# Pearbiossom-M/FlashAttention-from-Scratch-with-Triton

Hardware: AMD Instinct MI355X
Metric: achieved TFLOPS fwd and fwd+bwd (B=4,H=32,N=4096,D=64 causal); %MFMA peak (higher is better)
Workload: dtype bf16

## Files before the change

### flashattention-from-scratch-with-triton_amd/csrc/fa_api.hip

```cpp
#include <stdint.h>
#include <stdio.h>
#include <string.h>

#include <atomic>

#include "../../include/mi355fa.h"
#include "../../include/mi355fa_local.h"
#include "../../include/mi355fa_gqa.h"
#include "../../include/mi355fa_kvcache.h"
#include "../../include/mi355fa_softcap.h"
#include "../../include/mi355fa_alibi.h"
#include "../../include/mi355fa_kvcache_fp8.h"
#include "../../include/mi355fa_sink.h"
#include "../../include/mi355fa_paged.h"
#include "../../include/mi355fa_ragged.h"
#include "fa_decode.h"
#include "fa_kernels.h"

namespace fa {
std::atomic<int> g_force_fwd{0}, g_force_dq{0}, g_force_dkv{0};
std::atomic<int> g_force_kvsplits{0};
}

namespace {

thread_local char g_err[256] = "";
void* g_dbg = nullptr;

int fail(int code, const char* fmt, const char* what) {
  snprintf(g_err, sizeof(g_err), fmt, what);
  return code;
}

int hip_fail(hipError_t e, const char* what) {
  snprintf(g_err, sizeof(g_err), "%s: %s (%d)", what, hipGetErrorString(e), (int)e);
  return (int)e;
}

bool misaligned(const void* p) { return (reinterpret_cast<uintptr_t>(p) & 15u) != 0; }

int check_scale(const char* fn, float scale) {
  uint32_t u;
  memcpy(&u, &scale, sizeof(u));
  const bool negative_or_zero = (u >> 31) != 0 || (u & 0x7fffffffu) == 0;
  const bool nan_or_inf = ((u >> 23) & 0xffu) == 0xffu;
  if (negative_or_zero || nan_or_inf) return fail(MI355FA_ERR_SHAPE, "%s: scale must be finite and > 0", fn);
  return 0;
}

int check_softcap(const char* fn, float softcap) {
  uint32_t u;
  memcpy(&u, &softcap, sizeof(u));
  const bool negative_or_zero = (u >> 31) != 0 || (u & 0x7fffffffu) == 0;
  const bool nan_or_inf = ((u >> 23) & 0xffu) == 0xffu;
  if (negative_or_zero || nan_or_inf) return fail(MI355FA_ERR_SOFTCAP, "%s: softcap must be finite and > 0", fn);
  return 0;
}

int check_common(const char* fn, int B, int H, int Sq, int Sk, int D, int dtype, bool decode = false) {
  if (B < 1 || H < 1 || Sq < 1 || Sk < 1) return fail(MI355FA_ERR_SHAPE, "%s: B, H, S_q, S_k must be >= 1", fn);
  if (D != 64 && D != 128 && !(decode && D == 256)) return fail(MI355FA_ERR_HEAD_DIM, "%s: head dim must be 64 or 128", fn);
  if (dtype != MI355FA_FP16 && dtype != MI355FA_BF16) return fail(MI355FA_ERR_DTYPE, "%s: dtype must be 0 (fp16) or 1 (bf16)", fn);
  const long long lim = (1ll << 31) - 1;
  if ((long long)Sq * D * 2 > lim || (long long)Sk * D * 2 > lim)
    return fail(MI355FA_ERR_SHAPE, "%s: one (batch, head) slice exceeds 2^31 bytes", fn);
  if ((long long)B * H * ((Sq > Sk ? Sq : Sk) + 127) / 128 > lim)
    return fail(MI355FA_ERR_SHAPE, "%s: too many tiles for one launch", fn);
  return 0;
}

int make_layout(const char* fn, const long long* st, int H, int S, int D, fa::TensorLayout* out, int out_B = 0) {
  if (!st) {
    *out = fa::contiguous_layout(H, S, D);
    return 0;
// ... 34 lines not shown
  out->seed_hi = (unsigned)(seed >> 32);
  out->offset = (unsigned)offset;
  out->rp = 256.f / (256.f - (float)thresh);
  return 0;
}

}

__global__ __launch_bounds__(256, 1) void fa_poison_kernel() {
  extern __shared__ __attribute__((aligned(16))) char poison_smem[];
  const unsigned nan2 = 0x7FC07FC0u;
  for (int i = threadIdx.x; i < 160 * 1024 / 4; i += 256) ((unsigned*)poison_smem)[i] = nan2;
#define FA_P4(n) "v_mov_b32 v" #n ", %0\n\tv_accvgpr_write_b32 a" #n ", %0\n\t"
#define FA_P16(a, b, c, d) FA_P4(a) FA_P4(b) FA_P4(c) FA_P4(d)
  asm volatile(
      FA_P16(8, 9, 10, 11) FA_P16(12, 13, 14, 15) FA_P16(16, 17, 18, 19) FA_P16(20, 21, 22, 23) FA_P16(24, 25, 26, 27) FA_P16(28, 29, 30, 31)
      FA_P16(32, 33, 34, 35) FA_P16(36, 37, 38, 39) FA_P16(40, 41, 42, 43) FA_P16(44, 45, 46, 47) FA_P16(48, 49, 50, 51) FA_P16(52, 53, 54, 55)
      FA_P16(56, 57, 58, 59) FA_P16(60, 61, 62, 63) FA_P16(64, 65, 66, 67) FA_P16(68, 69, 70, 71) FA_P16(72, 73, 74, 75) FA_P16(76, 77, 78, 79)
      FA_P16(80, 81, 82, 83) FA_P16(84, 85, 86, 87) FA_P16(88, 89, 90, 91) FA_P16(92, 93, 94, 95) FA_P16(96, 97, 98, 99) FA_P16(100, 101, 102, 103)
      FA_P16(104, 105, 106, 107) FA_P16(108, 109, 110, 111) FA_P16(112, 113, 114, 115) FA_P16(116, 117, 118, 119) FA_P16(120, 121, 122, 123)
      FA_P16(124, 125, 126, 127) FA_P16(128, 129, 130, 131) FA_P16(132, 133, 134, 135) FA_P16(136, 137, 138, 139) FA_P16(140, 141, 142, 143)
      FA_P16(144, 145, 146, 147) FA_P16(148, 149, 150, 151) FA_P16(152, 153, 154, 155) FA_P16(156, 157, 158, 159) FA_P16(160, 161, 162, 163)
      FA_P16(164, 165, 166, 167) FA_P16(168, 169, 170, 171) FA_P16(172, 173, 174, 175) FA_P16(176, 177, 178, 179) FA_P16(180, 181, 182, 183)
      FA_P16(184, 185, 186, 187) FA_P16(188, 189, 190, 191) FA_P16(192, 193, 194, 195) FA_P16(196, 197, 198, 199) FA_P16(200, 201, 202, 203)
      FA_P16(204, 205, 206, 207) FA_P16(208, 209, 210, 211) FA_P16(212, 213, 214, 215) FA_P16(216, 217, 218, 219) FA_P16(220, 221, 222, 223)
      FA_P16(224, 225, 226, 227) FA_P16(228, 229, 230, 231) FA_P16(232, 233, 234, 235) FA_P16(236, 237, 238, 239) FA_P16(240, 241, 242, 243)
      FA_P16(244, 245, 246, 247) FA_P16(248, 249, 250, 251) FA_P16(252, 253, 254, 255)
      "v_accvgpr_write_b32 a0, %0\n\tv_accvgpr_write_b32 a1, %0\n\tv_accvgpr_write_b32 a2, %0\n\tv_accvgpr_write_b32 a3, %0\n\t"
      "v_accvgpr_write_b32 a4, %0\n\tv_accvgpr_write_b32 a5, %0\n\tv_accvgpr_write_b32 a6, %0\n\tv_accvgpr_write_b32 a7, %0"
      :: "v"(nan2)
      : "memory"
#define FA_C(n) , "v" #n, "a" #n
#define FA_C8(n) FA_C(n##0) FA_C(n##1) FA_C(n##2) FA_C(n##3) FA_C(n##4) FA_C(n##5) FA_C(n##6) FA_C(n##7) FA_C(n##8) FA_C(n##9)
        , "v8", "v9", "a0", "a1", "a2", "a3", "a4", "a5", "a6", "a7", "a8", "a9"
        FA_C8(1) FA_C8(2) FA_C8(3) FA_C8(4) FA_C8(5) FA_C8(6) FA_C8(7) FA_C8(8) FA_C8(9) FA_C8(10) FA_C8(11) FA_C8(12) FA_C8(13) FA_C8(14)
        FA_C8(15) FA_C8(16) FA_C8(17) FA_C8(18) FA_C8(19) FA_C8(20) FA_C8(21) FA_C8(22) FA_C8(23) FA_C8(24)
        FA_C(250) FA_C(251) FA_C(252) FA_C(253) FA_C(254) FA_C(255));
#undef FA_C8
#undef FA_C
#undef FA_P16
#undef FA_P4
  __syncthreads();
}

extern "C" {

int fa_abi_version(void) { return MI355FA_ABI_VERSION; }

void fa_debug_force_impl(int fwd, int dq, int dkv) {
  fa::g_force_fwd.store(fwd, std::memory_order_relaxed);
  fa::g_force_dq.store(dq, std::memory_order_relaxed);
  fa::g_force_dkv.store(dkv, std::memory_order_relaxed);
}

int fa_debug_pick(int kernel, int D, int dtype, int causal, int B, int H, int S_q, int S_k) {
  if (kernel == 0) return fa::pick_fwd_impl(fa::g_force_fwd, D, dtype, B, H, S_q, S_k, causal != 0, true);
  if (kernel == 1) return fa::pick_dq_impl(fa::g_force_dq, D, dtype, B, H, S_q, S_k, causal != 0);
  return fa::pick_dkv_impl(fa::g_force_dkv, D, dtype, B, H, S_q, S_k, causal != 0);
}

int fa_debug_pick_ex(int kernel, int D, int dtype, int causal, int B, int H, int S_q, int S_k, int varlen, int contiguous,
                     int dropout) {
  (void)contiguous;
  if (kernel == 0) return fa::fwd_family(D, dtype, B, H, S_q, S_k, causal != 0, varlen != 0, dropout != 0);
  if (kernel == 1) return fa::dq_family(D, dtype, B, H, S_q, S_k, causal != 0, varlen != 0, dropout != 0);
  return fa::dkv_family(D, dtype, B, H, S_q, S_k, causal != 0, varlen != 0, dropout != 0);
}

int fa_debug_fastdiv(int n, int d) {
  const fa::FastDiv f = fa::make_fastdiv(d);
  const unsigned hi = (unsigned)(((unsigned long long)f.m * (unsigned)n) >> 32);
  return (int)((hi + (unsigned)n) >> f.l);
}

void fa_debug_set_buffer(void* p) { g_dbg = p; }

int fa_debug_poison(void* stream) {
  return (int)fa::launch_kernel<fa_poison_kernel>(2048, 256, 160 * 1024, (hipStream_t)stream);
}

void fa_debug_kvcache_splits(int n) { fa::g_force_kvsplits.store(n > 0 ? n : 0, std::memory_order_relaxed); }

const char* fa_last_error(void) { return g_err; }

int fa_supported(int D, int dtype) {
  return (D == 64 || D == 128) && (dtype == MI355FA_FP16 || dtype == MI355FA_BF16);
}

static int check_sinks(const char* fn, const float* sinks) {
  if (!sinks) return fail(MI355FA_ERR_NULL, "%s: sinks is NULL", fn);
  if (reinterpret_cast<uintptr_t>(sinks) & 3u) return fail(MI355FA_ERR_ALIGN, "%s: sinks must be 4-byte aligned", fn);
  return 0;
}

static int check_alibi(const char* fn, const float* slopes, long long stride, int B, int H) {
  if (!slopes) return fail(MI355FA_ERR_NULL, "%s: alibi_slopes is NULL", fn);
  if (reinterpret_cast<uintptr_t>(slopes) & 3u) return fail(MI355FA_ERR_ALIGN, "%s: alibi_slopes must be 4-byte aligned", fn);
  if (stride < 0 || (stride > 0 && stride < (long long)H))
    return fail(MI355FA_ERR_ALIBI, "%s: slopes_batch_stride must be 0 (shape (H,)) or >= H (shape (B, H))", fn);
  if (stride > 0 && (long long)(B > 1 ? B - 1 : 0) * stride + H > 0x7fffffffLL)
    return fail(MI355FA_ERR_ALIBI, "%s: slopes_batch_stride too large: (B - 1) * stride + H must stay below 2^31", fn);
  return 0;
}

static int make_group(const char* fn, int H, int H_kv, fa::ScoreMod* w) {
  if (H_kv < 1 || (H >= 1 && H % H_kv != 0))
// ... 796 lines not shown
```

### flashattention-from-scratch-with-triton_amd/csrc/fa_bwd_dkv_v4.hip

```cpp
#include <stdlib.h>

#include <type_traits>

#include "fa_common.h"
#include "fa_kernels.h"
#include "fa_stamps.h"

namespace fa {

struct Dkv4Cfg : Ring4Cfg<64, 128, 3> {
  static constexpr int D = 64;
  static constexpr int BK = 256, BQ = TILE_ROWS, NT = 256, NW = 4;
  static constexpr int QB = BQ / 32;
  static constexpr int ROWB = D * 2, CPR = D / 8, KS = D / 16, DB = D / 32;
  static constexpr int QBLK = 32 * ROWB;
  static constexpr int DO_BASE = NBUF * TILE_BYTES;
  static constexpr int ROWC_OFF = 2 * NBUF * TILE_BYTES;
  static constexpr int ROWC_BYTES = 2 * BQ * 4;
  static constexpr int KS_OFF = ROWC_OFF + NBUF * ROWC_BYTES;
  static constexpr int KG_BYTES = 32 * ROWB;
  static constexpr int EPI_OFF = KS_OFF + BK * ROWB;
  static constexpr int LDS_BYTES = EPI_OFF + NW * KG_BYTES;
  static constexpr int NS = 16;
  static constexpr int ACC_DV = 0, ACC_DK = 64, F_K = 16, F_V = 24, A_RC = 192;
  static constexpr int STAGE_PIECES = KG_BYTES / 1024;
  static constexpr int kStageReqs = 4 * STAGE_PIECES;
  static constexpr int kRowConstReqs = kPfLoadReqs;
  static constexpr int kPrologueReqs = 2 * kTileReqs + kRowConstReqs;
  static constexpr int kEpilogueStores = 4 * kTileRowStores<D>;
};


template <typename T, bool CAUSAL>
__global__ __launch_bounds__(256, 1) void fa_bwd_dkv4_kernel(BwdParams p) {
#ifdef FA_STAMPS
  FA_STAMPS_BEGIN(8);
  unsigned long long ntile_ = 0, npass_ = 0;
#endif
  using C = Dkv4Cfg;
  using vec8 = typename T::vec8;
  constexpr int D = C::D;
  constexpr bool FOLD = T::kFoldScale;
  extern __shared__ __attribute__((aligned(16))) char smem_raw[];
  FA_LDS char* smem = (FA_LDS char*)smem_raw;

  const int tid = threadIdx.x;
  const int wave = __builtin_amdgcn_readfirstlane(tid >> 6);

  const bool paired = CAUSAL && p.pair;
  const int nk = p.n_tiles;
  const int per_bh = paired ? (nk + 1) / 2 : nk;
  const int n_items = per_bh * p.B * p.H;
  const int Sq = p.Sq, Sk = p.Sk;
  const int q_rs = p.lq.rs, do_rs = p.ldo.rs, kv_rs = p.lk.rs;
  const float c2 = p.scale * kLog2e;
  const int lds0 = (int)lds_addr_of(smem);
  const int ntiles = Sq / C::BQ;
  const bool rc_lse = wave < 2;
  pin_reserve();

  struct Work {
    int b, h, idx, npass;
  };
  auto decode = [&](int item) __attribute__((always_inline)) -> Work {
    const int w = xcd_remap(item, n_items);
    const int bh = p.div_per_bh.div(w), idx = w - bh * per_bh, b = p.div_h.div(bh);
    return Work{b, bh - b * p.H, idx, (paired && idx != nk - 1 - idx) ? 2 : 1};
  };
  auto ktile_of = [&](const Work& wk, int pass) __attribute__((always_inline)) -> int {
    return paired ? (pass == 0 ? wk.idx : nk - 1 - wk.idx) : wk.idx;
  };
  struct Stage {
    __amdgpu_buffer_rsrc_t rk, rv;
    int key0[2];
  };
  auto stage_of = [&](const Work& wk, int pass, bool valid) __attribute__((always_inline)) -> Stage {
    const int k0 = ktile_of(wk, pass) * C::BK;
    const unsigned nb = valid ? view_bytes(Sk, kv_rs, C::ROWB) : 0u;
    return Stage{make_rsrc((const char*)p.k + wk.b * p.lk.sb + wk.h * p.lk.sh, nb),
                 make_rsrc((const char*)p.v + wk.b * p.lv.sb + wk.h * p.lv.sh, nb), {k0 + 32 * wave, k0 + 32 * (7 - wave)}};
  };
  auto stage_group = [&](const Stage& st, int vslot, int g) __attribute__((always_inline)) {
    const int ln = lane_id_now(), prow = ln >> 3;
    const int kg = g & 1;
    int voff[C::STAGE_PIECES];
#pragma unroll
    for (int i = 0; i < C::STAGE_PIECES; ++i)
      voff[i] = (st.key0[kg] + 8 * i + prow) * kv_rs + swz_chunk<D>(8 * i + prow, ln & 7) * 16 - 1024 * i;
    const int dst = g < 2 ? C::KS_OFF + (2 * wave + kg) * C::KG_BYTES : (kg ? C::DO_BASE : 0) + vslot * C::TILE_BYTES + wave * C::KG_BYTES;
    dma_pieces<C::STAGE_PIECES>(g < 2 ? st.rk : st.rv, (unsigned)(lds0 + dst), voff, 0);
  };

  int item = blockIdx.x;
  Work wk = decode(item);
  Work nwk_item = decode(min(item + (int)gridDim.x, n_items - 1));
  int b0 = 0, b1 = 1, b2 = 2;
  bool staged = false;
  for (; item < n_items; item += gridDim.x, wk = nwk_item, nwk_item = decode(min(item + (int)gridDim.x, n_items - 1))) {
  const int b_ = wk.b, h_ = wk.h, npass = wk.npass;
  const __amdgpu_buffer_rsrc_t rq = make_rsrc((const char*)p.q + b_ * p.lq.sb + h_ * p.lq.sh, view_bytes(Sq, q_rs, C::ROWB));
  const __amdgpu_buffer_rsrc_t rdo = make_rsrc((const char*)p.dout + b_ * p.ldo.sb + h_ * p.ldo.sh, view_bytes(Sq, do_rs, C::ROWB));
  const __amdgpu_buffer_rsrc_t rrc = make_rsrc((rc_lse ? p.lse : p.delta) + b_ * p.lse_sb + h_ * p.lse_sh, (unsigned)Sq * 4);

  for (int pass = 0; pass < npass; ++pass) {
    const int lane = lane_id_now(), r = lane & 31, h = lane >> 5;
    const int k0_wg = ktile_of(wk, pass) * C::BK;
    const int kw[2] = {k0_wg + 32 * wave, k0_wg + 32 * (7 - wave)};
    const int t0 = CAUSAL ? k0_wg / C::BQ : 0;
    const int n_main = CAUSAL ? ntiles - t0 - 2 : ntiles, n_pos = n_main + (CAUSAL ? 2 : 0);
    auto tile_at = [&](int i) __attribute__((always_inline)) -> int {
      if constexpr (CAUSAL) return i < n_main ? t0 + 2 + i : (i < n_pos ? t0 + i - n_main : -1);
      return i < n_main ? i : -1;
    };

    int dma_q[C::PIECES], dma_do[C::PIECES];
#pragma unroll
    for (int i = 0; i < C::PIECES; ++i) {
      const int row = (C::BQ / C::NW) * wave + C::RPI * i + lane / C::CPR;
      const int chunk = swz_chunk<D>(row, lane % C::CPR) * 16;
      dma_q[i] = row * q_rs + chunk - 1024 * (i & 1);
      dma_do[i] = row * do_rs + chunk - 1024 * (i & 1);
    }
    auto dma_tile = [&](__amdgpu_buffer_rsrc_t rq_, __amdgpu_buffer_rsrc_t rdo_, int t, int buf, int g4) __attribute__((always_inline)) {
      static_assert(4 * 2 == C::kTileReqs, "a tile goes out as four groups of dma_pieces<2>");
      const int i = 2 * (g4 & 1);
      const int dst = buf * C::TILE_BYTES + ((C::BQ / C::NW) * wave + C::RPI * i) * C::ROWB;
      const int sq = t >= 0 ? t * C::BQ * q_rs : C::kOOB, sd = t >= 0 ? t * C::BQ * do_rs : C::kOOB;
      if (g4 < 2) dma_pieces<2>(rq_, (unsigned)(lds0 + dst), dma_q + i, sq);
      else dma_pieces<2>(rdo_, (unsigned)(lds0 + C::DO_BASE + dst), dma_do + i, sd);
    };
    auto dma_group = [&](int pos, int buf, int g4) __attribute__((always_inline)) { dma_tile(rq, rdo, tile_at(pos), buf, g4); };
    auto rc_tile = [&](__amdgpu_buffer_rsrc_t rrc_, auto a_tag, int t) __attribute__((always_inline)) {
      int x;
      asm volatile("v_and_b32 %0, %1, %2" : "=v"(x) : "n"(C::BQ - 1), "v"(tid));
      pf_load4<decltype(a_tag)::value>(rrc_, t >= 0 ? (t * C::BQ + x) * 4 : C::kOOB);
    };
    auto rc_request = [&](auto a_tag, int pos) __attribute__((always_inline)) { rc_tile(rrc, a_tag, tile_at(pos)); };
    auto rc_publish = [&](auto a_tag, int buf) __attribute__((always_inline)) {
      const float v = acc_read1<decltype(a_tag)::value>();
      FA_LDS float* rcp = (FA_LDS float*)(smem + C::ROWC_OFF + buf * C::ROWC_BYTES);
      rcp[tid] = rc_lse ? -v * kLog2e : -v;
    };
    using RC0 = std::integral_constant<int, C::A_RC>;
    using RC1 = std::integral_constant<int, C::A_RC + 1>;

    if (!staged) {
      const Stage st = stage_of(wk, pass, true);
#pragma unroll
      for (int g = 0; g < 4; ++g) stage_group(st, b2, g);
      asm volatile("s_waitcnt vmcnt(0)" ::: "memory");
#pragma unroll
      for (int g4 = 0; g4 < 4; ++g4) dma_group(0, b0, g4);
#pragma unroll
      for (int g4 = 0; g4 < 4; ++g4) dma_group(1, b1, g4);
      rc_request(RC0{}, 0);
    } else {
      constexpr int kYounger = C::kPrologueReqs + C::kEpilogueStores;
      static_assert(kYounger == 2 * C::kTileReqs + kPfLoadReqs + 4 * kTileRowStores<D>,
                    "two tiles and one rc_tile in front of the epilogue, four store_tile_rows in it");
      static_assert(kYounger == 33 && vmcnt_fits(kYounger), "counted wait");
      asm volatile("s_waitcnt vmcnt(%0)" ::"n"(kYounger) : "memory");
    }
    int row_off[C::KS];
#pragma unroll
    for (int ks = 0; ks < C::KS; ++ks) row_off[ks] = lds_off<D>(r, 2 * ks + h);
    static_for<2 * C::KS>([&](auto i_) __attribute__((always_inline)) {
      constexpr int i = decltype(i_)::value, g = i / C::KS, ks = i % C::KS;
      vec8 kk = as_vec8<T>(lds_read16(smem + C::KS_OFF + (2 * wave + g) * C::KG_BYTES + row_off[ks]));
      if (FOLD && !p.q_prescaled) kk = scale_frag<T>(kk, c2);
      pin_write<C::F_K + 4 * g + ks>(__builtin_bit_cast(u32x4, kk));
      pin_write<C::F_V + 4 * g + ks>(lds_read16(smem + (g ? C::DO_BASE : 0) + b2 * C::TILE_BYTES + wave * C::KG_BYTES + row_off[ks]));
    });
    __builtin_amdgcn_sched_barrier(0);
    static_for<8>([](auto i_) __attribute__((always_inline)) { acc_zero16<16 * decltype(i_)::value>(); });

    int tr_off[2][C::DB];
#pragma unroll
    for (int e = 0; e < 2; ++e)
#pragma unroll
      for (int db = 0; db < C::DB; ++db) tr_off[e][db] = tr_lane_off<D>(lane, 8 * e, db);

    f32x16 S_[2], P_[2];
    f32x16 NL[FOLD ? 1 : 2], ND;
    f32x16 CD;
    u32x4 RF[8];
    vec8 TF[8];
    u32x4 pk[2][2], sk[2][2];

    auto block_valu = [&](int tau, f32x16& X, f32x16& Y, u32x4 (&pkb)[2], u32x4 (&skb)[2], const f32x16& nl) __attribute__((always_inline)) {
      const int e = tau - 5, m = tau - 10;
      if (e >= 0 && e < 16) {
        float x = here(X[e]);
        if constexpr (!FOLD) x = __builtin_fmaf(x, c2, nl[e]);
        X[e] = __builtin_amdgcn_exp2f(x);
      }
      if (m >= 0 && m < 16) Y[m] = X[m] * Y[m];
      if (tau >= 7 && tau <= 21 && ((tau - 7) & 1) == 0) {
        const int j = (tau - 7) >> 1;
        pkb[j >> 2][j & 3] = pack2<T>(X[2 * j], X[2 * j + 1]);
      }
// ... 101 lines not shown
#pragma unroll
      for (int ks = 0; ks < C::KS; ++ks) {
        RF[ks] = lds_read16(smem + off + row_off[ks]);
        RF[4 + ks] = lds_read16(smem + C::DO_BASE + off + row_off[ks]);
      }
#pragma unroll
      for (int q = 0; q < 4; ++q) {
        const f32x4 a = *(const FA_LDS f32x4*)(smem + rc_off + (8 * q + 4 * h) * 4);
        const f32x4 d = *(const FA_LDS f32x4*)(smem + rc_off + (C::BQ + 8 * q + 4 * h) * 4);
#pragma unroll
        for (int j = 0; j < 4; ++j) {
          NL[FOLD ? 0 : par][4 * q + j] = a[j];
          ND[4 * q + j] = d[j];
        }
      }
    };
    auto pipe_fill = [&](auto pg_tag, int prev_par) __attribute__((always_inline)) {
      constexpr int PG = decltype(pg_tag)::value;
      const unsigned lz = (unsigned)lane_id_now() >> 6;
      const float lzf = __builtin_bit_cast(float, lz);
#pragma unroll
      for (int i = 0; i < 16; ++i) {
        S_[PG][i] = i < 11 ? lzf : -INFINITY + lzf;
        P_[PG][i] = lzf;
        if (!FOLD) NL[FOLD ? 0 : (prev_par & 1)][i] = lzf;
      }
#pragma unroll
      for (int e = 0; e < 2; ++e) {
        pk[PG][e] = u32x4{lz, lz, lz, lz};
        sk[PG][e] = u32x4{lz, lz, lz, lz};
      }
#pragma unroll
      for (int n = 0; n < 8; ++n) TF[n] = as_vec8<T>(u32x4{lz, lz, lz, lz});
    };

    asm volatile("s_waitcnt vmcnt(0)" ::: "memory");
    rc_publish(RC0{}, b0);
    rc_request(RC0{}, 1);
    dma_group(2, b2, 0);
    dma_group(2, b2, 1);
    asm volatile("s_nop 4");
    __builtin_amdgcn_s_waitcnt(waitcnt_imm(kNoWait, 0));
    __builtin_amdgcn_s_barrier();
    asm volatile("" ::: "memory");

    load_block(b0 * C::TILE_BYTES, C::ROWC_OFF + b0 * C::ROWC_BYTES, 0);
    pipe_fill(I1{}, 1);
    __builtin_amdgcn_sched_barrier(0);

    FA_STAMP(0);
    const bool nc_stage = !CAUSAL && item + (int)gridDim.x < n_items && n_main >= 3;
    auto tile_step = [&](int i, auto sel_tag) __attribute__((always_inline)) {
      constexpr int SEL = decltype(sel_tag)::value;
      const Stage est = stage_of(nwk_item, 0, SEL != 0);
#ifdef FA_STAMPS
      ++ntile_;
#endif
      int tA[2][C::DB], kq[C::KS], kN[C::KS];
      tr_bases(tA, tr_off, lds0, b0 * C::TILE_BYTES);
      row_bases(kq, row_off, lds0, b0 * C::TILE_BYTES);
      row_bases(kN, row_off, lds0, b1 * C::TILE_BYTES);
      const int rcA = opaque(lds0 + C::ROWC_OFF + b0 * C::ROWC_BYTES + 16 * h), rcN = opaque(lds0 + C::ROWC_OFF + b1 * C::ROWC_BYTES + 16 * h);
      auto hook_first = [&](int s, int phase) __attribute__((always_inline)) {
        if constexpr (SEL == 0 || SEL == 1) {
          if (phase == 1 && s == 9) dma_group(i + 2, b2, 2);
          if (phase == 1 && s == 13) dma_group(i + 2, b2, 3);
        } else if constexpr (SEL == 2) {
          if (phase == 1 && s == 9) stage_group(est, b2, 0);
          if (phase == 1 && s == 13) stage_group(est, b2, 1);
        }
      };
      auto hook_last = [&](int s, int phase) __attribute__((always_inline)) {
        if (phase == 0 && s == 4) {
          constexpr int kYounger = SEL == 2 ? C::kStageReqs : C::kTileReqs;
          static_assert(C::kTileReqs == 8 && C::kStageReqs == 16 && vmcnt_fits(kYounger), "counted wait");
          static_assert(C::kStageReqs == C::kTileReqs + 2 * C::STAGE_PIECES, "SEL 2: a staging pair in each half tile's slots");
          asm volatile("s_waitcnt vmcnt(%0)" ::"n"(kYounger) : "memory");
          rc_publish(RC0{}, b1);
          __builtin_amdgcn_s_waitcnt(waitcnt_imm(kNoWait, 0));
          __builtin_amdgcn_s_barrier();
          asm volatile("" ::: "memory");
          rc_request(RC0{}, i + 2);
        }
        if constexpr (SEL == 0) {
          if (phase == 1 && s == 9) dma_group(i + 3, b0, 0);
          if (phase == 1 && s == 13) dma_group(i + 3, b0, 1);
        } else if constexpr (SEL == 1) {
          if (phase == 1 && s == 9) stage_group(est, b0, 2);
          if (phase == 1 && s == 13) stage_group(est, b0, 3);
        }
      };
      block_iter(I0{}, I0{}, I1{}, I0{}, No{}, No{}, No{}, tA, 0 * C::QBLK, kq, 0, 0, hook_first);
      block_iter(I1{}, I1{}, I0{}, I0{}, No{}, Yes{}, No{}, tA, 0 * C::QBLK, kq, 1 * C::QBLK, rcA + 1 * 32 * 4, no_hook);
      block_iter(I0{}, I0{}, I1{}, I1{}, No{}, No{}, No{}, tA, 1 * C::QBLK, kq, 0, 0, no_hook);
      block_iter(I1{}, I1{}, I0{}, I1{}, No{}, Yes{}, No{}, tA, 1 * C::QBLK, kq, 2 * C::QBLK, rcA + 2 * 32 * 4, no_hook);
      block_iter(I0{}, I0{}, I1{}, I0{}, No{}, No{}, No{}, tA, 2 * C::QBLK, kq, 0, 0, no_hook);
      block_iter(I1{}, I1{}, I0{}, I0{}, No{}, Yes{}, No{}, tA, 2 * C::QBLK, kq, 3 * C::QBLK, rcA + 3 * 32 * 4, no_hook);
      block_iter(I0{}, I0{}, I1{}, I1{}, No{}, No{}, No{}, tA, 3 * C::QBLK, kq, 0, 0, no_hook);
      block_iter(I1{}, I1{}, I0{}, I1{}, No{}, Yes{}, No{}, tA, 3 * C::QBLK, kN, 0, rcN, hook_last);
      ring_rotate(b0, b1, b2);
    };
    {
      int i = 0;
      const int nmain = nc_stage ? n_main - 3 : n_main;
      for (; i < nmain; ++i) tile_step(i, I0{});
      if constexpr (!CAUSAL) {
        if (nc_stage) {
          tile_step(i, I1{});
          tile_step(i + 1, std::integral_constant<int, 2>{});
          tile_step(i + 2, std::integral_constant<int, 3>{});
        }
      }
    }

    FA_STAMP(1);
    if constexpr (!CAUSAL) {
      pipe_drain(I1{}, I1{}, I1{});
      if (nc_stage) ring_rotate(b0, b1, b2);
      staged = nc_stage;
    } else {
      asm volatile("s_waitcnt vmcnt(0)" ::: "memory");
      rc_publish(RC0{}, b1);
      __builtin_amdgcn_s_waitcnt(waitcnt_imm(kNoWait, 0));
      __builtin_amdgcn_s_barrier();
      asm volatile("" ::: "memory");
      auto qbase = [&](int q) __attribute__((always_inline)) {
        return (q < C::QB ? b0 * C::TILE_BYTES : b1 * C::TILE_BYTES - C::QB * C::QBLK) + q * C::QBLK;
      };
      auto rcaddr = [&](int q) __attribute__((always_inline)) {
        return lds0 + C::ROWC_OFF + (q < C::QB ? b0 : b1) * C::ROWC_BYTES + (q & (C::QB - 1)) * 32 * 4 + 16 * h;
      };
      auto diag_start = [&](int par) __attribute__((always_inline)) {
#pragma unroll
        for (int i = 0; i < 16; ++i) CD[i] = (r > (i & 3) + 8 * (i >> 2) + 4 * h) ? -INFINITY : (FOLD ? NL[0][i] : 0.f);
        (void)par;
        settle_mfma(CD);
      };
      static_assert(FOLD, "the causal instance exists for the folded-scale dtype only (launch_bwd_dkv_v4)");
      const bool more_pass = pass + 1 < npass, more_item = item + (int)gridDim.x < n_items;
      const Stage nst = stage_of(more_pass ? wk : nwk_item, more_pass ? pass + 1 : 0,
                                 more_pass || more_item);
      auto hook_a = [&](int s, int phase) __attribute__((always_inline)) {
        if (phase == 1 && s == 2) stage_group(nst, b2, 0);
        if (phase == 1 && s == 10) stage_group(nst, b2, 1);
      };
      auto hook_b = [&](int s, int phase) __attribute__((always_inline)) {
        if (phase == 1 && s == 6) stage_group(nst, b2, 2);
      };
      auto hook_c = [&](int s, int phase) __attribute__((always_inline)) {
        if (phase == 1 && s == 4) stage_group(nst, b2, 3);
      };
      staged = more_pass || more_item;
      int trb[2][C::DB], nxt[C::KS];
      load_block(qbase(7), rcaddr(7) - lds0 - 16 * h, 1);
      __builtin_amdgcn_sched_barrier(0);
      int q = 7;
      for (; q > 7 - wave; --q) {
        tr_bases(trb, tr_off, lds0, qbase(q));
        row_bases(nxt, row_off, lds0, qbase(q - 1));
        block_iter(I0{}, I0{}, I1{}, I0{}, No{}, No{}, No{}, trb, 0, nxt, 0, 0, no_hook);
        block_iter(I1{}, I1{}, I0{}, I0{}, No{}, Yes{}, No{}, trb, 0, nxt, 0, rcaddr(q - 1), no_hook);
      }
      tr_bases(trb, tr_off, lds0, qbase(q));
      row_bases(nxt, row_off, lds0, qbase(max(q - 1, 0)));
      block_iter(I0{}, I0{}, I1{}, I0{}, No{}, No{}, No{}, trb, 0, nxt, 0, 0, hook_a);
      diag_start(q);
      block_iter(I1{}, I1{}, I0{}, I0{}, No{}, Yes{}, Yes{}, trb, 0, nxt, 0, rcaddr(max(q - 1, 0)), hook_b);
      auto solo = [&](auto g_tag, auto pkg_tag, auto next_tag, auto diag_tag, int off, int off_next, int rc_next, auto&& hook) __attribute__((always_inline)) {
        tr_bases(trb, tr_off, lds0, off);
        if constexpr (decltype(next_tag)::value) row_bases(nxt, row_off, lds0, off_next);
        if constexpr (decltype(diag_tag)::value) diag_start(0);
        block_iter(g_tag, I0{}, pkg_tag, I0{}, Yes{}, next_tag, diag_tag, trb, 0, nxt, 0, rc_next, hook);
      };
      if (6 - wave <= wave) {
        solo(I0{}, I1{}, No{}, Yes{}, qbase(wave), 0, 0, hook_c);
      } else {
        q = 6 - wave;
        solo(I0{}, I1{}, Yes{}, No{}, qbase(q), qbase(q - 1), rcaddr(q - 1), no_hook);
        for (q = 5 - wave; q > wave + 1; q -= 2) {
          solo(I1{}, I0{}, Yes{}, No{}, qbase(q), qbase(q - 1), rcaddr(q - 1), no_hook);
          solo(I0{}, I0{}, Yes{}, No{}, qbase(q - 1), qbase(q - 2), rcaddr(q - 2), no_hook);
        }
        solo(I1{}, I0{}, Yes{}, No{}, qbase(wave + 1), qbase(wave), rcaddr(wave), no_hook);
        solo(I0{}, I0{}, No{}, Yes{}, qbase(wave), 0, 0, hook_c);
      }
      FA_STAMP(2);
      pipe_drain(I0{}, I0{}, I0{});
    }
    FA_STAMP(3);
    if constexpr (!CAUSAL) {
      if (!staged) asm volatile("s_waitcnt vmcnt(0)" ::: "memory");
    }

    __syncthreads();
    {
      if (staged) {
        const bool more_pass = pass + 1 < npass;
        const Work nw = more_pass ? wk : nwk_item;
        const int t0n = ktile_of(nw, more_pass ? pass + 1 : 0) * C::BK / C::BQ, n_mainn = ntiles - t0n - 2;
        const int tn0 = !CAUSAL ? 0 : (n_mainn > 0 ? t0n + 2 : t0n), tn1 = !CAUSAL ? 1 : (n_mainn > 1 ? t0n + 3 : (n_mainn == 1 ? t0n : t0n + 1));
        const __amdgpu_buffer_rsrc_t nrq = make_rsrc((const char*)p.q + nw.b * p.lq.sb + nw.h * p.lq.sh, view_bytes(Sq, q_rs, C::ROWB));
        const __amdgpu_buffer_rsrc_t nrdo = make_rsrc((const char*)p.dout + nw.b * p.ldo.sb + nw.h * p.ldo.sh, view_bytes(Sq, do_rs, C::ROWB));
        const __amdgpu_buffer_rsrc_t nrrc = make_rsrc((rc_lse ? p.lse : p.delta) + nw.b * p.lse_sb + nw.h * p.lse_sh, (unsigned)Sq * 4);
#pragma unroll
        for (int g4 = 0; g4 < 4; ++g4) dma_tile(nrq, nrdo, tn0, b0, g4);
#pragma unroll
        for (int g4 = 0; g4 < 4; ++g4) dma_tile(nrq, nrdo, tn1, b1, g4);
        rc_tile(nrrc, RC0{}, tn0);
      }
    }
    FA_LDS char* stage = smem + C::EPI_OFF + wave * C::KG_BYTES;
    const float dk_mul = (FOLD && p.q_prescaled) ? kLn2 : p.scale;
    {
      const int dk_rs = p.ldk.rs, dv_rs = p.ldv.rs;
      const __amdgpu_buffer_rsrc_t rdk = make_rsrc((char*)p.dk + b_ * p.ldk.sb + h_ * p.ldk.sh, view_bytes(Sk, dk_rs, C::ROWB));
      const __amdgpu_buffer_rsrc_t rdv = make_rsrc((char*)p.dv + b_ * p.ldv.sb + h_ * p.ldv.sh, view_bytes(Sk, dv_rs, C::ROWB));
      const f32x16 dk0[C::DB] = {acc_read16<C::ACC_DK>(), acc_read16<C::ACC_DK + 16>()};
      store_tile_rows<D, T>(dk0, dk_mul, stage, rdk, kw[0] * dk_rs, lane, dk_rs);
      const f32x16 dv0[C::DB] = {acc_read16<C::ACC_DV>(), acc_read16<C::ACC_DV + 16>()};
      store_tile_rows<D, T>(dv0, 1.0f, stage, rdv, kw[0] * dv_rs, lane, dv_rs);
      const f32x16 dk1[C::DB] = {acc_read16<C::ACC_DK + 32>(), acc_read16<C::ACC_DK + 48>()};
      store_tile_rows<D, T>(dk1, dk_mul, stage, rdk, kw[1] * dk_rs, lane, dk_rs);
      const f32x16 dv1[C::DB] = {acc_read16<C::ACC_DV + 32>(), acc_read16<C::ACC_DV + 48>()};
      store_tile_rows<D, T>(dv1, 1.0f, stage, rdv, kw[1] * dv_rs, lane, dv_rs);
    }
    FA_STAMP(4);
#ifdef FA_STAMPS
    ++npass_;
#endif
  }
  }
#ifdef FA_STAMPS
  if (p.dbg && (threadIdx.x & 63) == 0) {
    unsigned long long* d = stamp_record(p.dbg, wave, 32);
    for (int i = 0; i < 8; ++i) d[i] = seg[i];
    d[17] = ntile_;
    FA_STAMPS_END(d, 18);
    d[20] = npass_;
  }
#endif
}

template <typename T, bool CAUSAL>
static hipError_t launch4(const BwdParams& p, hipStream_t s) {
  using C = Dkv4Cfg;
  int grid = (CAUSAL && p.pair ? (p.n_tiles + 1) / 2 : p.n_tiles) * p.B * p.H;
  grid = persistent_grid(grid);
  return launch_kernel<fa_bwd_dkv4_kernel<T, CAUSAL>>(grid, C::NT, C::LDS_BYTES, s, p);
}

hipError_t launch_bwd_dkv_v4(BwdParams p, int dtype, int causal, hipStream_t s) {
  p.n_tiles = (p.Sk + Dkv4Cfg::BK - 1) / Dkv4Cfg::BK;
  p.pair = want_pairs(causal != 0, p.n_tiles, (long)p.B * p.H);
  p.div_per_bh = make_fastdiv(p.pair ? (p.n_tiles + 1) / 2 : p.n_tiles);
  p.div_h = make_fastdiv(p.H);
  if (dtype == 1) return causal ? launch4<BF16, true>(p, s) : launch4<BF16, false>(p, s);
  return causal ? hipErrorInvalidValue : launch4<FP16, false>(p, s);
}

}
```

### flashattention-from-scratch-with-triton_amd/csrc/fa_kernels.h

```cpp
#pragma once
#include <hip/hip_runtime.h>

#include <atomic>

#include "fa_table.h"

namespace fa {

struct TensorLayout {
  long long sb, sh;
  int rs;
};
inline TensorLayout contiguous_layout(int H, int S, int D) {
  return TensorLayout{(long long)H * S * D * 2, (long long)S * D * 2, D * 2};
}

struct FastDiv {
  unsigned m;
  int l;
  __device__ __forceinline__ int div(int n) const { return (int)((__umulhi(m, (unsigned)n) + (unsigned)n) >> l); }
};
inline FastDiv make_fastdiv(int d) {
  int l = 0;
  while ((1ll << l) < d) ++l;
// ... 5 lines not shown
  const int* cu_k;
};

struct DropoutParams {
  unsigned thresh, seed_lo, seed_hi, offset;
  float rp;
};

struct SeqInfo {
  int q0, k0, Sq, Sk;
};
__device__ __forceinline__ SeqInfo seq_info(const VarLen& vl, int b, int Sq, int Sk) {
  if (!vl.cu_q) return SeqInfo{0, 0, Sq, Sk};
  const int q0 = vl.cu_q[b], q1 = vl.cu_q[b + 1], k0 = vl.cu_k[b], k1 = vl.cu_k[b + 1];
  return SeqInfo{q0, k0, q1 - q0, k1 - k0};
}

struct FwdParams {
  const void* q;
  const void* k;
  const void* v;
  void* o;
  float* lse;
  int B, H, Sq, Sk;
  float scale;
  int nq_tiles;
  void* dbg;
  int pair;
  FastDiv div_per_bh, div_h;
  TensorLayout lq, lk, lv;
  TensorLayout lo;
  long long lse_sb, lse_sh;
  VarLen vl;
  DropoutParams drop;
};

struct BwdParams {
  const void* q;
  const void* k;
  const void* v;
  const void* o;
  const void* dout;
  const float* lse;
  float* delta;
  void* dq;
  void* dk;
  void* dv;
  int B, H, Sq, Sk;
  float scale;
  int n_tiles;
  void* dbg;
  int pair;
  FastDiv div_per_bh, div_h;
  TensorLayout lq, lk, lv, ldo;
  TensorLayout lo, ldq, ldk, ldv;
  void* qs;
  TensorLayout lqs;
  int q_prescaled;
  long long lse_sb, lse_sh;
  VarLen vl;
  DropoutParams drop;
};

struct BatchHead {
  int b, h;
};
__device__ __forceinline__ BatchHead batch_head(int slice, int B, int H, bool varlen) {
  if (varlen) {
    const int h = slice / B;
    return BatchHead{slice - h * B, h};
  }
  const int b = slice / H;
  return BatchHead{b, slice - b * H};
}

__device__ __forceinline__ int xcd_remap(int b, int n) {
  const int q = n >> 3, r = n & 7, x = b & 7, idx = b >> 3;
  return (x < r ? x * (q + 1) : r * (q + 1) + (x - r) * q) + idx;
}
template <bool CAUSAL>
struct TileIndex {
  int pair;
  int bh, idx;
  __device__ __forceinline__ bool paired() const { return CAUSAL && pair; }
  __device__ __forceinline__ bool surplus(int n) const { return idx >= (paired() ? (n + 1) / 2 : n); }
  __device__ __forceinline__ int npass(int n) const { return (paired() && idx != n - 1 - idx) ? 2 : 1; }
  __device__ __forceinline__ int qtile(int n, int pass) const { return paired() ? (pass == 0 ? n - 1 - idx : idx) : (CAUSAL ? n - 1 - idx : idx); }
};
template <bool CAUSAL, typename P>
__device__ __forceinline__ TileIndex<CAUSAL> tile_index_of(const P& p, int w, int per_bh) {
  const int bh = w / per_bh;
  return TileIndex<CAUSAL>{p.pair, bh, w - bh * per_bh};
}
template <bool CAUSAL, typename P>
__device__ __forceinline__ TileIndex<CAUSAL> tile_index(const P& p, const int& n_tiles) {
  const int w = xcd_remap(blockIdx.x, gridDim.x);
  const bool paired = CAUSAL && p.pair;
  const int per_bh = paired ? (n_tiles + 1) / 2 : n_tiles;
  return tile_index_of<CAUSAL>(p, w, per_bh);
}
template <bool CAUSAL, typename P>
__device__ __forceinline__ TileIndex<CAUSAL> tile_index_item(const P& p, int item, int n_items, int per_bh) {
  return tile_index_of<CAUSAL>(p, xcd_remap(item, n_items), per_bh);
}
inline hipError_t opt_in_lds(const void* kern, int bytes, std::atomic<unsigned long long>& done) {
  int dev = 0;
  hipError_t e = hipGetDevice(&dev);
  if (e != hipSuccess) return e;
  const unsigned long long bit = dev < 64 ? 1ull << dev : 0;
  if (bit && (done.load(std::memory_order_relaxed) & bit)) return hipSuccess;
  e = hipFuncSetAttribute(kern, hipFuncAttributeMaxDynamicSharedMemorySize, bytes);
  if (e == hipSuccess) done.fetch_or(bit, std::memory_order_relaxed);
  return e;
}

template <auto Kern, typename... Args>
hipError_t launch_kernel(unsigned grid, int block, int lds, hipStream_t s, Args... args) {
  if (lds > 48 * 1024) {
    static std::atomic<unsigned long long> opted_in{0};
    if (hipError_t e = opt_in_lds((const void*)Kern, lds, opted_in)) return e;
  }
  hipLaunchKernelGGL(Kern, dim3(grid), dim3(block), lds, s, args...);
  return hipGetLastError();
}
inline int persistent_grid(int items) {
  static std::atomic<int> cus{0};
  int n = cus.load(std::memory_order_relaxed);
  if (n == 0) {
    int dev = 0;
    if (hipGetDevice(&dev) != hipSuccess || hipDeviceGetAttribute(&n, hipDeviceAttributeMultiprocessorCount, dev) != hipSuccess || n < 8) n = 256;
    n -= n % 8;
    cus.store(n, std::memory_order_relaxed);
  }
  return items < n ? items : n;
}
template <int D, int ROWS, int NBUF_>
struct Ring4Cfg {
  static constexpr int TILE_ROWS = ROWS, NBUF = NBUF_;
  static constexpr int TILE_BYTES = ROWS * D * 2;
  static constexpr int PIECES = TILE_BYTES / (4 * 1024);
  static constexpr int RPI = 1024 / (D * 2);
  static constexpr int kOOB = 0x7FFFFFFF;
  static constexpr int kTileReqs = 2 * PIECES;
};

extern std::atomic<int> g_force_fwd, g_force_dq, g_force_dkv;

inline int nearest_log2_bucket(long v, const int* buckets, int n) {
  int best = 0;
  for (int i = 1; i < n; ++i)
    if ((double)v * v > (double)buckets[i - 1] * buckets[i]) best = i;
  return best;
}
enum { kKernelFwd = 0, kKernelDq = 1, kKernelDkv = 2 };
inline int table_family(int kernel, int D, int dtype, bool causal, long bh, long S) {
  if (D != 64 && D != 128) return 1;
  return table::kFamily[kernel][D == 128][dtype == 1][causal ? 1 : 0][nearest_log2_bucket(bh, table::kBH, table::kNumBH)]
// ... 55 lines not shown
```

Measured before the change: 888.4.

## Precompute per-block work items in lane registers for dkv kernel persistent loop

Replaces per-iteration decode (fastdiv, xcd remap, stride multiplies) of work items in the persistent dK/dV kernel with a lane-distributed worklist. It decodes up to 63 future items in parallel across wave lanes, along with precomputed base offsets, and reads them back with readlane. The aim is to take scalar index and address arithmetic off the critical path between tiles. In exchange it adds VGPR pressure for the cached tag and offsets, and adds readlane overhead.

```diff
diff --git a/flashattention-from-scratch-with-triton_amd/csrc/fa_api.hip b/flashattention-from-scratch-with-triton_amd/csrc/fa_api.hip
--- a/flashattention-from-scratch-with-triton_amd/csrc/fa_api.hip
+++ b/flashattention-from-scratch-with-triton_amd/csrc/fa_api.hip
@@ -20,6 +20,7 @@
 namespace fa {
 std::atomic<int> g_force_fwd{0}, g_force_dq{0}, g_force_dkv{0};
 std::atomic<int> g_force_kvsplits{0};
+std::atomic<int> g_worklist_chunk{0};
 }
 
 namespace {
@@ -160,6 +161,8 @@
   fa::g_force_dq.store(dq, std::memory_order_relaxed);
   fa::g_force_dkv.store(dkv, std::memory_order_relaxed);
 }
+
+void fa_debug_set_worklist_chunk(int n) { fa::g_worklist_chunk.store(n, std::memory_order_relaxed); }
 
 int fa_debug_pick(int kernel, int D, int dtype, int causal, int B, int H, int S_q, int S_k) {
   if (kernel == 0) return fa::pick_fwd_impl(fa::g_force_fwd, D, dtype, B, H, S_q, S_k, causal != 0, true);
diff --git a/flashattention-from-scratch-with-triton_amd/csrc/fa_bwd_dkv_v4.hip b/flashattention-from-scratch-with-triton_amd/csrc/fa_bwd_dkv_v4.hip
--- a/flashattention-from-scratch-with-triton_amd/csrc/fa_bwd_dkv_v4.hip
+++ b/flashattention-from-scratch-with-triton_amd/csrc/fa_bwd_dkv_v4.hip
@@ -34,7 +34,7 @@
 template <typename T, bool CAUSAL>
 __global__ __launch_bounds__(256, 1) void fa_bwd_dkv4_kernel(BwdParams p) {
 #ifdef FA_STAMPS
-  FA_STAMPS_BEGIN(8);
+  FA_STAMPS_BEGIN(9);
   unsigned long long ntile_ = 0, npass_ = 0;
 #endif
   using C = Dkv4Cfg;
@@ -48,6 +48,7 @@
   const int wave = __builtin_amdgcn_readfirstlane(tid >> 6);
 
   const bool paired = CAUSAL && p.pair;
+  const bool uni = (p.worklist & kWorkUniform) != 0;
   const int nk = p.n_tiles;
   const int per_bh = paired ? (nk + 1) / 2 : nk;
   const int n_items = per_bh * p.B * p.H;
@@ -59,9 +60,6 @@
   const bool rc_lse = wave < 2;
   pin_reserve();
 
-  struct Work {
-    int b, h, idx, npass;
-  };
   auto decode = [&](int item) __attribute__((always_inline)) -> Work {
     const int w = xcd_remap(item, n_items);
     const int bh = p.div_per_bh.div(w), idx = w - bh * per_bh, b = p.div_h.div(bh);
@@ -77,8 +75,8 @@
   auto stage_of = [&](const Work& wk, int pass, bool valid) __attribute__((always_inline)) -> Stage {
     const int k0 = ktile_of(wk, pass) * C::BK;
     const unsigned nb = valid ? view_bytes(Sk, kv_rs, C::ROWB) : 0u;
-    return Stage{make_rsrc((const char*)p.k + wk.b * p.lk.sb + wk.h * p.lk.sh, nb),
-                 make_rsrc((const char*)p.v + wk.b * p.lv.sb + wk.h * p.lv.sh, nb), {k0 + 32 * wave, k0 + 32 * (7 - wave)}};
+    return Stage{make_rsrc(work_base(uni, (const char*)p.k, wk, wk.ok, p.lk.sb, p.lk.sh), nb),
+                 make_rsrc(work_base(uni, (const char*)p.v, wk, wk.ok, p.lv.sb, p.lv.sh), nb), {k0 + 32 * wave, k0 + 32 * (7 - wave)}};
   };
   auto stage_group = [&](const Stage& st, int vslot, int g) __attribute__((always_inline)) {
     const int ln = lane_id_now(), prow = ln >> 3;
@@ -91,16 +89,19 @@
     dma_pieces<C::STAGE_PIECES>(g < 2 ? st.rk : st.rv, (unsigned)(lds0 + dst), voff, 0);
   };
 
+  const WorkStrides wstr{p.lq.sb, p.lq.sh, p.lk.sb, p.lk.sh, 4 * p.lse_sb, 4 * p.lse_sh};
+  WorkList wl;
+  wl.begin(p.worklist, wstr, n_items, decode);
+  FA_STAMP(8);
   int item = blockIdx.x;
-  Work wk = decode(item);
-  Work nwk_item = decode(min(item + (int)gridDim.x, n_items - 1));
   int b0 = 0, b1 = 1, b2 = 2;
   bool staged = false;
-  for (; item < n_items; item += gridDim.x, wk = nwk_item, nwk_item = decode(min(item + (int)gridDim.x, n_items - 1))) {
-  const int b_ = wk.b, h_ = wk.h, npass = wk.npass;
-  const __amdgpu_buffer_rsrc_t rq = make_rsrc((const char*)p.q + b_ * p.lq.sb + h_ * p.lq.sh, view_bytes(Sq, q_rs, C::ROWB));
-  const __amdgpu_buffer_rsrc_t rdo = make_rsrc((const char*)p.dout + b_ * p.ldo.sb + h_ * p.ldo.sh, view_bytes(Sq, do_rs, C::ROWB));
-  const __amdgpu_buffer_rsrc_t rrc = make_rsrc((rc_lse ? p.lse : p.delta) + b_ * p.lse_sb + h_ * p.lse_sh, (unsigned)Sq * 4);
+  for (; item < n_items; item += gridDim.x, wl.advance(wstr, n_items, decode)) {
+  const Work wk = wl.at(false);
+  const int npass = wk.npass;
+  const __amdgpu_buffer_rsrc_t rq = make_rsrc(work_base(uni, (const char*)p.q, wk, wk.oq, p.lq.sb, p.lq.sh), view_bytes(Sq, q_rs, C::ROWB));
+  const __amdgpu_buffer_rsrc_t rdo = make_rsrc(work_base(uni, (const char*)p.dout, wk, wk.oq, p.ldo.sb, p.ldo.sh), view_bytes(Sq, do_rs, C::ROWB));
+  const __amdgpu_buffer_rsrc_t rrc = make_rsrc(work_base(uni, rc_lse ? p.lse : p.delta, wk, wk.ol, 4 * p.lse_sb, 4 * p.lse_sh), (unsigned)Sq * 4);
 
   for (int pass = 0; pass < npass; ++pass) {
     const int lane = lane_id_now(), r = lane & 31, h = lane >> 5;
@@ -145,7 +146,7 @@
     using RC1 = std::integral_constant<int, C::A_RC + 1>;
 
     if (!staged) {
-      const Stage st = stage_of(wk, pass, true);
+      const Stage st = stage_of(wl.at(false), pass, true);
 #pragma unroll
       for (int g = 0; g < 4; ++g) stage_group(st, b2, g);
       asm volatile("s_waitcnt vmcnt(0)" ::: "memory");
@@ -353,7 +354,7 @@
     const bool nc_stage = !CAUSAL && item + (int)gridDim.x < n_items && n_main >= 3;
     auto tile_step = [&](int i, auto sel_tag) __attribute__((always_inline)) {
       constexpr int SEL = decltype(sel_tag)::value;
-      const Stage est = stage_of(nwk_item, 0, SEL != 0);
+      const Stage est = stage_of(wl.at(true), 0, SEL != 0);
 #ifdef FA_STAMPS
       ++ntile_;
 #endif
@@ -439,8 +440,7 @@
       };
       static_assert(FOLD, "the causal instance exists for the folded-scale dtype only (launch_bwd_dkv_v4)");
       const bool more_pass = pass + 1 < npass, more_item = item + (int)gridDim.x < n_items;
-      const Stage nst = stage_of(more_pass ? wk : nwk_item, more_pass ? pass + 1 : 0,
-                                 more_pass || more_item);
+      const Stage nst = stage_of(wl.at(!more_pass), more_pass ? pass + 1 : 0, more_pass || more_item);
       auto hook_a = [&](int s, int phase) __attribute__((always_inline)) {
         if (phase == 1 && s == 2) stage_group(nst, b2, 0);
         if (phase == 1 && s == 10) stage_group(nst, b2, 1);
@@ -497,12 +497,12 @@
     {
       if (staged) {
         const bool more_pass = pass + 1 < npass;
-        const Work nw = more_pass ? wk : nwk_item;
+        const Work nw = wl.at(!more_pass);
         const int t0n = ktile_of(nw, more_pass ? pass + 1 : 0) * C::BK / C::BQ, n_mainn = ntiles - t0n - 2;
         const int tn0 = !CAUSAL ? 0 : (n_mainn > 0 ? t0n + 2 : t0n), tn1 = !CAUSAL ? 1 : (n_mainn > 1 ? t0n + 3 : (n_mainn == 1 ? t0n : t0n + 1));
-        const __amdgpu_buffer_rsrc_t nrq = make_rsrc((const char*)p.q + nw.b * p.lq.sb + nw.h * p.lq.sh, view_bytes(Sq, q_rs, C::ROWB));
-        const __amdgpu_buffer_rsrc_t nrdo = make_rsrc((const char*)p.dout + nw.b * p.ldo.sb + nw.h * p.ldo.sh, view_bytes(Sq, do_rs, C::ROWB));
-        const __amdgpu_buffer_rsrc_t nrrc = make_rsrc((rc_lse ? p.lse : p.delta) + nw.b * p.lse_sb + nw.h * p.lse_sh, (unsigned)Sq * 4);
+        const __amdgpu_buffer_rsrc_t nrq = make_rsrc(work_base(uni, (const char*)p.q, nw, nw.oq, p.lq.sb, p.lq.sh), view_bytes(Sq, q_rs, C::ROWB));
+        const __amdgpu_buffer_rsrc_t nrdo = make_rsrc(work_base(uni, (const char*)p.dout, nw, nw.oq, p.ldo.sb, p.ldo.sh), view_bytes(Sq, do_rs, C::ROWB));
+        const __amdgpu_buffer_rsrc_t nrrc = make_rsrc(work_base(uni, rc_lse ? p.lse : p.delta, nw, nw.ol, 4 * p.lse_sb, 4 * p.lse_sh), (unsigned)Sq * 4);
 #pragma unroll
         for (int g4 = 0; g4 < 4; ++g4) dma_tile(nrq, nrdo, tn0, b0, g4);
 #pragma unroll
@@ -514,8 +514,9 @@
     const float dk_mul = (FOLD && p.q_prescaled) ? kLn2 : p.scale;
     {
       const int dk_rs = p.ldk.rs, dv_rs = p.ldv.rs;
-      const __amdgpu_buffer_rsrc_t rdk = make_rsrc((char*)p.dk + b_ * p.ldk.sb + h_ * p.ldk.sh, view_bytes(Sk, dk_rs, C::ROWB));
-      const __amdgpu_buffer_rsrc_t rdv = make_rsrc((char*)p.dv + b_ * p.ldv.sb + h_ * p.ldv.sh, view_bytes(Sk, dv_rs, C::ROWB));
+      const Work ew = wl.at(false);
+      const __amdgpu_buffer_rsrc_t rdk = make_rsrc(work_base(uni, (char*)p.dk, ew, ew.ok, p.ldk.sb, p.ldk.sh), view_bytes(Sk, dk_rs, C::ROWB));
+      const __amdgpu_buffer_rsrc_t rdv = make_rsrc(work_base(uni, (char*)p.dv, ew, ew.ok, p.ldv.sb, p.ldv.sh), view_bytes(Sk, dv_rs, C::ROWB));
       const f32x16 dk0[C::DB] = {acc_read16<C::ACC_DK>(), acc_read16<C::ACC_DK + 16>()};
       store_tile_rows<D, T>(dk0, dk_mul, stage, rdk, kw[0] * dk_rs, lane, dk_rs);
       const f32x16 dv0[C::DB] = {acc_read16<C::ACC_DV>(), acc_read16<C::ACC_DV + 16>()};
@@ -538,6 +539,7 @@
     d[17] = ntile_;
     FA_STAMPS_END(d, 18);
     d[20] = npass_;
+    d[21] = seg[8];
   }
 #endif
 }
@@ -555,6 +557,8 @@
   p.pair = want_pairs(causal != 0, p.n_tiles, (long)p.B * p.H);
   p.div_per_bh = make_fastdiv(p.pair ? (p.n_tiles + 1) / 2 : p.n_tiles);
   p.div_h = make_fastdiv(p.H);
+  const bool uni = uniform_strides(p.lq, p.ldo) && uniform_strides(p.lk, p.lv) && uniform_strides(p.lk, p.ldk) && uniform_strides(p.lk, p.ldv);
+  p.worklist = worklist_chunk() | (uni ? kWorkUniform : 0);
   if (dtype == 1) return causal ? launch4<BF16, true>(p, s) : launch4<BF16, false>(p, s);
   return causal ? hipErrorInvalidValue : launch4<FP16, false>(p, s);
 }
diff --git a/flashattention-from-scratch-with-triton_amd/csrc/fa_kernels.h b/flashattention-from-scratch-with-triton_amd/csrc/fa_kernels.h
--- a/flashattention-from-scratch-with-triton_amd/csrc/fa_kernels.h
+++ b/flashattention-from-scratch-with-triton_amd/csrc/fa_kernels.h
@@ -81,6 +81,7 @@
   void* dbg;
   int pair;
   FastDiv div_per_bh, div_h;
+  int worklist;
   TensorLayout lq, lk, lv, ldo;
   TensorLayout lo, ldq, ldk, ldv;
   void* qs;
@@ -132,6 +133,71 @@
 __device__ __forceinline__ TileIndex<CAUSAL> tile_index_item(const P& p, int item, int n_items, int per_bh) {
   return tile_index_of<CAUSAL>(p, xcd_remap(item, n_items), per_bh);
 }
+struct Work {
+  int b, h, idx, npass;
+  long long oq, ok, ol;
+};
+struct WorkStrides {
+  long long qb, qh, kb, kh, lb, lh;
+};
+constexpr int kWorkUniform = 0x100;
+inline bool uniform_strides(const TensorLayout& a, const TensorLayout& b) { return a.sb == b.sb && a.sh == b.sh; }
+extern std::atomic<int> g_worklist_chunk;
+inline int worklist_chunk() {
+  const int n = g_worklist_chunk.load(std::memory_order_relaxed);
+  return n >= 1 && n < 63 ? n : 63;
+}
+struct WorkList {
+  long long oq, ok, ol;
+  int tag;
+  int k, end, chunk;
+  bool uni;
+  template <typename F>
+  __device__ __forceinline__ void fill(int k0, const WorkStrides& s, int n_items, F&& decode) {
+    const int lane = (int)__builtin_amdgcn_mbcnt_hi(~0u, __builtin_amdgcn_mbcnt_lo(~0u, 0u));
+    const int j = (lane - k0) & 63;
+    const long long it = (long long)blockIdx.x + (long long)(k0 + j) * (long long)gridDim.x;
+    const Work w = decode((int)(it < n_items - 1 ? it : n_items - 1));
+    if (j < chunk) {
+      tag = w.idx | (w.npass << 24);
+      oq = uni ? w.b * s.qb + w.h * s.qh : (long long)(((unsigned long long)(unsigned)w.h << 32) | (unsigned)w.b);
+      ok = w.b * s.kb + w.h * s.kh;
+      ol = w.b * s.lb + w.h * s.lh;
+    }
+    end = k0 + chunk;
+  }
+  template <typename F>
+  __device__ __forceinline__ void begin(int worklist, const WorkStrides& s, int n_items, F&& decode) {
+    k = 0;
+    chunk = worklist & 63;
+    uni = (worklist & kWorkUniform) != 0;
+    tag = 0, oq = ok = ol = 0;
+    fill(0, s, n_items, decode);
+    if (end < 2) fill(1, s, n_items, decode);
+  }
+  template <typename F>
+  __device__ __forceinline__ void advance(const WorkStrides& s, int n_items, F&& decode) {
+    ++k;
+    if (k + 1 >= end) fill(k + 1, s, n_items, decode);
+  }
+  __device__ __forceinline__ Work at(bool next) const {
+    const int l = (k + (next ? 1 : 0)) & 63;
+    const int t = __builtin_amdgcn_readlane(tag, l);
+    auto rd64 = [&](long long v) __attribute__((always_inline)) {
+      const unsigned lo = (unsigned)__builtin_amdgcn_readlane((int)(unsigned)v, l);
+      const unsigned hi = (unsigned)__builtin_amdgcn_readlane((int)(unsigned)((unsigned long long)v >> 32), l);
+      return (long long)(((unsigned long long)hi << 32) | lo);
+    };
+    const long long q = rd64(oq);
+    return Work{(int)(unsigned)q, (int)(unsigned)((unsigned long long)q >> 32), t & 0xffffff, t >> 24, q, rd64(ok), rd64(ol)};
+  }
+};
+template <typename P>
+__device__ __forceinline__ P* work_base(bool uni, P* ptr, const Work& w, long long off, long long sb, long long sh) {
+  if (uni) return (P*)((char*)ptr + off);
+  return (P*)((char*)ptr + (w.b * sb + w.h * sh));
+}
+
 inline hipError_t opt_in_lds(const void* kern, int bytes, std::atomic<unsigned long long>& done) {
   int dev = 0;
   hipError_t e = hipGetDevice(&dev);
```

Measured after the change: 889.7 (median of 3 runs). About the same (+0.1%).
